# SKIRT/SKIRT9

Measured on AMD Instinct MI355X. Metric: photon packets/s (whole node), 10^6-cell octree, higher is better.
Workload: dtype f64

## Files before the change

skirt9_amd/csrc/pmc_context.h:

```cpp
#ifndef PMC_CONTEXT_H
#define PMC_CONTEXT_H

#include "pmc_device.h"
#include "../../include/pmc_layout.h"
#include "../../include/pmc_tuning.h"
#include <hip/hip_runtime.h>
#include <algorithm>
#include <chrono>
#include <cmath>
#include <cstdio>
#include <rccl/rccl.h>
#include <cstdlib>
#include <cstring>
#include <deque>
#include <atomic>
#include <mutex>
#include <string>
#include <thread>
#include <map>
#include <vector>

extern "C" const char* pmcTune(const char* name);
extern "C" hipError_t pmcUploadScene(int slot, const DevScene* scene, hipStream_t stream);
extern "C" hipError_t pmcConfigureKernels(size_t walkLds, size_t transitionLds);
extern "C" int pmcWalkBlocksPerCU(int gridKind, int kind, int wide, int block, size_t ldsBytes);
extern "C" hipError_t pmcLaunchStatMerge(int slot, int blocks, hipStream_t stream);
extern "C" int pmcPeelBlock(void);
extern "C" int pmcPropBlock(void);
extern "C" hipError_t pmcLaunchWalk(int slot, int gridKind, int flavour, int taskBase, int numTaskRecords, int taskCounter, uint64_t seed, int grid,
                                    int block, size_t ldsBytes, const WalkStreamArgs* tasks, hipStream_t stream);
extern "C" hipError_t pmcLaunchPeel(int slot, int form, int slotBase, int numSlots, const int* list, int cursor, int obs, int sgn, int grid, size_t ldsBytes,
                                    const PeelRec* sortedRec, const unsigned long long* sortedCount, unsigned long long* xcdCursor, hipStream_t stream);
extern "C" int pmcVoroPropWavesPerSimd(void);
extern "C" hipError_t pmcLaunchVoroProp(int slot, const int32_t* list, const unsigned long long* count, unsigned long long* xcdCursor, int segments, uint64_t seed,
                                        int flavour, int grid, hipStream_t stream);
extern "C" int pmcVoroPeelWavesPerSimd(void);
extern "C" hipError_t pmcLaunchVoroPeel(int slot, int rec, int tab, const int32_t* list, const unsigned long long* count, unsigned long long* xcdCursor, int segments,
                                        int severalMedia, int grid, hipStream_t stream);
extern "C" hipError_t pmcLaunchProp(int slot, int wide, int flavour, int checkpoints, int slotBase, int numSlots, const int* list, int cursor, uint64_t seed,
                                    int grid, size_t ldsBytes, const RfLogArgs* rfLog, hipStream_t stream);
extern "C" hipError_t pmcLaunchRfFlush(int slot, const uint32_t* keys, const double* vals, uint32_t* sortedKeys, double* sortedVals, unsigned long long n,
                                       int numParts, void* temp, int numCU, hipStream_t stream);
extern "C" int pmcPeelHasQueues(int form, size_t ldsBytes);
extern "C" int pmcPropHasCheckpoints(int flavour, size_t ldsBytes);
extern "C" int pmcExperimentBuild(void);
extern "C" const unsigned long long* pmcPeelSortedCount(void* temp);
extern "C" size_t pmcPeelSortTempBytes();
extern "C" hipError_t pmcLaunchPeelSortCounts(int slot, int slotBase, int numSlots, PeelSortArgs* ps, PeelRec* const* sorted, int32_t* const* lists, void* const* temp,
                                              int* groups, hipStream_t stream);
extern "C" size_t pmcRfTempBytes(int numParts);
extern "C" int pmcRfMaxParts();
extern "C" hipError_t pmcLaunchDipoleCosines(const double* u, int64_t n, double* out, hipStream_t stream);
extern "C" hipError_t pmcLaunchSourceVelocities(int slot, int source, const double* r, int64_t n, double* out, hipStream_t stream);
extern "C" hipError_t pmcLaunchTransition(int slot, int flavour, int slotBase, int numSlots, int group, uint64_t seed, const int* list, int listLen, int maxBlocks,
                                          size_t ldsBytes, const StatLogArgs* statLog, uint64_t count, hipStream_t stream);
extern "C" hipError_t pmcLaunchLaunch(int slot, int kin, int slotBase, int numSlots, int group, uint64_t first, uint64_t count, uint64_t seed, int initial,
                                      int maxBlocks, size_t ldsBytes, const StatLogArgs* statLog, hipStream_t stream);
extern "C" hipError_t pmcLaunchStatFlush(int slot, const uint32_t* keys, const double* vals, uint32_t* sortedKeys, double* sortedVals, unsigned long long n,
                                         int numParts, void* temp, int numCU, const uint32_t* chunkFill, hipStream_t stream);
extern "C" int pmcStatBucketBits();
extern "C" hipError_t pmcLaunchCycleStart(int slot, int gridKind, int kin, int slotBase, int numSlots, int listCounter, int* listOut, const int* listIn,
                                          int listLen, int maxBlocks, size_t ldsBytes, const PeelSortArgs* sort, hipStream_t stream);
extern "C" hipError_t pmcLaunchTrace(int slot, int gridKind, int wide, int uniform, const double r[3], const double k[3],
                                     const double* kdev, int32_t* m, double* ds, int32_t cap, int32_t* n, size_t ldsBytes,
                                     hipStream_t stream);

void pmcSetError(const std::string& message);
namespace
{
    inline int fail(int code, const std::string& message)
    {
        pmcSetError(message);
        return code;
    }
    inline int hipFail(hipError_t e, const char* what)
    {
        return fail(PMC_ERR_DEVICE, std::string(what) + ": " + hipGetErrorString(e));
    }
}

#define HIP_TRY(call)                                           \
    do                                                          \
// ... 134 lines not shown
```

skirt9_amd/csrc/pmc_device.h:

```cpp
#ifndef PMC_DEVICE_H
#define PMC_DEVICE_H

#include "../../include/pmc.h"
#include <stdint.h>

#define PMC_MAX_INSTRUMENTS 16
#define PMC_MAX_CONTEXTS 6
#define PMC_MAX_LEVEL 20
#define PMC_STAT_CAP 48
#define PMC_STAT_EMISSION_BIN 0x20000000
#define PMC_STAT_POOL_EXHAUSTED 0x40000000

#define PMC_LINK_NONE 0x7FFFFFFFu
#define PMC_LINK_NODE 0x80000000u
#define PMC_LINK_OCTET 0x40000000u
#define PMC_LINK_EXP_BITS 5
#define PMC_LINK_EXP_MASK 31u
#define PMC_LINK_INDEX_MASK 0x1FFFFFFu
#define PMC_LINK_MAX_INDEX ((1u << 25) - 2u)

struct CellRec
{
    double   density;
    uint32_t link[6];
// ... 317 lines not shown
    const unsigned long long* count;
    unsigned long long* xcdCursor;
};
#ifndef PMC_PEEL_TILES
#define PMC_PEEL_TILES 32
#endif
#define PMC_VORO_RUN_UNIT_BITS 27
#define PMC_VORO_RUN_UNIT_MASK 0x07FFFFFFu
#define PMC_VORO_RUN_COUNT_UNKNOWN 31u
#define PMC_VORO_FIRST_SCAN (-1000)
#define PMC_VORO_RUN_PAD 16
#ifndef PMC_VORO_RUN_LANES
#define PMC_VORO_RUN_LANES 2
#endif
#ifndef PMC_VORO_CONES
#define PMC_VORO_CONES 192
#endif
#define PMC_RF_LOG_CHUNK 4096
#define PMC_RF_BUCKET_BITS 13

#define PMC_NUM_COUNTERS 512
#define PMC_CTR_HISTORY 8
#define PMC_CTR_WALKWORK 16
#define PMC_CTR_LIVE(g) (35 + 4 * (g))
#define PMC_CTR_TASK(g, k) (256 + 32 * (g) + (k))
#define PMC_CTR_TASKS_PER_GROUP 32
#define PMC_CTR_LIST(g) PMC_CTR_TASK(g, 30)
#define PMC_CTR_RFLOG(g) PMC_CTR_TASK(g, 31)
#define PMC_CTR_STATLOG(g) (56 + (g))
#define PMC_CTR_HBASE(g) (120 + (g))
#define PMC_CTR_HLIMIT(g) (124 + (g))
#define PMC_MAX_GROUPS 4
#define PMC_CTR_STATFREE(g) (48 + (g))
#define PMC_TRANSITION_ALIGN 1024

#endif
```

skirt9_amd/csrc/pmc_kernels.hip:

```cpp

#include "pmc_device.h"
#include "../../include/pmc_philox.h"
#include <hip/hip_runtime.h>
#include <cstdlib>
#include <cstring>
#include <float.h>
#include <math.h>
#include <algorithm>
#include <mutex>
#include <array>
#include <type_traits>
#include <utility>

#ifndef PMC_WALK_REFILL
    #define PMC_WALK_REFILL 40
#endif
#ifndef PMC_PEEL_REFILL
    #define PMC_PEEL_REFILL 32
#endif
#ifndef PMC_PROP_REFILL
    #define PMC_PROP_REFILL 40
#endif
#ifndef PMC_PEEL_BLOCK
    #define PMC_PEEL_BLOCK 768
// ... 329 lines not shown
{
    WalkStreamArgs ws;
    std::memset(&ws, 0, sizeof(ws));
    if (tasks) ws = *tasks;
    const WalkKernel kernel = gridKind == PMC_GRID_BINTREE ? binWalkKernels[flavour & 7].kernel : walkKernels[(flavour & 7) | (gridKind == PMC_GRID_VORONOI ? 8 : 0)].kernel;
    hipLaunchKernelGGL(kernel, dim3(grid), dim3(block), ldsBytes, stream, slot, taskBase, numTaskRecords, taskCounter, seed, ws);
    return hipGetLastError();
}

extern "C" int pmcVoroPeelWavesPerSimd(void) { return PMC_VPEEL_MIN_WAVES; }
extern "C" hipError_t pmcLaunchVoroPeel(int slot, int rec, int tab, const int32_t* list, const unsigned long long* count, unsigned long long* xcdCursor, int segments,
                                        int severalMedia, int grid, hipStream_t stream)
{
    hipLaunchKernelGGL(severalMedia ? voroPeelKernel<true> : voroPeelKernel<false>, dim3(grid), dim3(256), 0, stream, slot, rec, tab, list, count, xcdCursor,
                       segments);
    return hipGetLastError();
}

extern "C" int pmcVoroPropWavesPerSimd(void) { return PMC_VPROP_MIN_WAVES; }
extern "C" hipError_t pmcLaunchVoroProp(int slot, const int32_t* list, const unsigned long long* count, unsigned long long* xcdCursor, int segments, uint64_t seed,
                                        int flavour, int grid, hipStream_t stream)
{
    hipLaunchKernelGGL(voroPropKernels[flavour & 7], dim3(grid), dim3(256), 0, stream, slot, list, count, xcdCursor, segments, seed);
    return hipGetLastError();
}

constexpr int PEEL_SORT_GROUPS = 1024;
constexpr int PEEL_SORT_PARTS = PMC_PEEL_TILES * PMC_PEEL_TILES;
extern "C" size_t pmcPeelSortTempBytes()
{
    return (size_t(2) * PEEL_SORT_PARTS + 2) * sizeof(unsigned long long) + size_t(PEEL_SORT_GROUPS) * PEEL_SORT_PARTS * sizeof(uint32_t);
}
extern "C" const unsigned long long* pmcPeelSortedCount(void* temp) { return static_cast<const unsigned long long*>(temp) + 2 * PEEL_SORT_PARTS; }
extern "C" hipError_t pmcLaunchPeelSortCounts(int slot, int slotBase, int numSlots, PeelSortArgs* ps, PeelRec* const* sorted, int32_t* const* lists, void* const* temp,
                                              int* groups, hipStream_t stream)
{
    ps->numParts = PEEL_SORT_PARTS;
    const int numLists = ps->numObs + (ps->propIndex >= 0 ? 1 : 0);
    for (int k = 0; k < numLists; ++k)
    {
        unsigned long long* totals = static_cast<unsigned long long*>(temp[k]);
        ps->out[k] = sorted ? sorted[k] : nullptr;
        ps->listOut[k] = lists ? lists[k] : nullptr;
        ps->matrix[k] = reinterpret_cast<uint32_t*>(totals + 2 * PEEL_SORT_PARTS + 2);
        ps->start[k] = totals + PEEL_SORT_PARTS;
    }
    const int tiles = (numSlots + PEEL_SORT_TILE - 1) / PEEL_SORT_TILE;
    *groups = std::max(1, std::min(tiles, PEEL_SORT_GROUPS));
    hipLaunchKernelGGL(peelSortCountKernel, dim3(*groups), dim3(256), 0, stream, slot, slotBase, numSlots, *ps);
    for (int k = 0; k < numLists; ++k)
    {
        unsigned long long* totals = static_cast<unsigned long long*>(temp[k]);
        hipLaunchKernelGGL(peelSortOffsetsKernel, dim3((PEEL_SORT_PARTS + 15) / 16), dim3(256), 0, stream, ps->matrix[k], (uint32_t)*groups, (uint32_t)PEEL_SORT_PARTS, totals);
        hipLaunchKernelGGL(rfScanKernel, dim3(1), dim3(PMC_SCAN_THREADS), 0, stream, totals, totals + PEEL_SORT_PARTS, (uint32_t)PEEL_SORT_PARTS);
    }
    return hipGetLastError();
}

extern "C" hipError_t pmcLaunchPeel(int slot, int form, int slotBase, int numSlots, const int* list, int cursor, int obs, int sgn, int grid, size_t ldsBytes,
                                    const PeelRec* sortedRec, const unsigned long long* sortedCount, unsigned long long* xcdCursor, hipStream_t stream)
{
    if (!(form & 4))
        hipLaunchKernelGGL(peelKernels[form & 3].kernel, dim3(grid), dim3(PMC_PEEL_BLOCK), ldsBytes, stream, slot, slotBase, numSlots, cursor, obs, list);
    else
    {
        const size_t queueOffset = (ldsBytes + 15) & ~size_t(15);
        const PeelSortedArgs sorted = {sortedRec, sortedCount, xcdCursor};
        hipLaunchKernelGGL(peel2Kernels[(form & 1) * 8 + (sgn & 7)].kernel, dim3(grid), dim3(PMC_PEEL_BLOCK), queueOffset + pmcPeelQueueBytes(), stream, slot,
                           slotBase, numSlots, cursor, obs, (int)queueOffset, list, sorted);
    }
    return hipGetLastError();
}

extern "C" hipError_t pmcLaunchProp(int slot, int wide, int flavour, int checkpoints, int slotBase, int numSlots, const int* list, int cursor, uint64_t seed,
                                    int grid, size_t ldsBytes, const RfLogArgs* rfLog, hipStream_t stream)
{
    const PropKernel kernel = propKernels[(flavour & 7) | (wide ? 8 : 0)].kernel;
    const size_t trimOffset = (ldsBytes + 15) & ~size_t(15);
    RfLogArgs none = {nullptr, nullptr, 0ull, 0, 0u};
    hipLaunchKernelGGL(kernel, dim3(grid), dim3(PMC_PROP_BLOCK), checkpoints ? trimOffset + PROP_CKPT_BYTES : ldsBytes, stream, slot, slotBase, numSlots, cursor,
                       seed, checkpoints ? (int)trimOffset : -1, rfLog ? *rfLog : none, list);
    return hipGetLastError();
// ... 146 lines not shown
```

skirt9_amd/csrc/pmc_run.hip:

```cpp
#include "pmc_context.h"

namespace
{
    int allocateSlotArrays(pmc_ctx* ctx, int64_t n);
    void releaseSlots(pmc_ctx* ctx)
    {
        for (void* p : ctx->slotAllocations) hipFree(p);
        ctx->slotAllocations.clear();
        ctx->allocatedSlots = 0;
    }

    int allocateSlots(pmc_ctx* ctx, int64_t n)
    {
        hipSetDevice(ctx->device);
        releaseSlots(ctx);
        ctx->planning = true;
        ctx->plannedBytes = 0;
        int rc = allocateSlotArrays(ctx, n);
        ctx->planning = false;
        if (rc) return rc;
        size_t freeBytes = 0, totalBytes = 0;
        if (!ctx->slotsConfigured && n > (int64_t(1) << 20) && hipMemGetInfo(&freeBytes, &totalBytes) == hipSuccess && ctx->plannedBytes > freeBytes / 2)
        {
            const int64_t less = std::max<int64_t>(int64_t(1) << 20, n / 2);
// ... 100 lines not shown
        for (int32_t** d : tints)
            if ((rc = ctx->allocate<int32_t>(nt, d, false, &own))) return rc;
        if ((rc = ctx->allocate<uint32_t>(size_t(n) / 64 + 64, &K.endedCount, true, &own))) return rc;
        if ((rc = ctx->allocate<int32_t>(2 * size_t(n), &K.liveList, false, &own))) return rc;
        if ((rc = ctx->allocate<uint32_t>(nt, &K.bits, false, &own))) return rc;
    if (ctx->dev.grid_kind == PMC_GRID_OCTREE && (rc = ctx->allocate<uint64_t>(nt, &K.pidx, false, &own))) return rc;
        if (ctx->planning) return PMC_OK;
        A.num_slots = n;
        ctx->allocatedSlots = n;
        ctx->sceneDirty = true;
        return PMC_OK;
    }
}

int pmcAllocateSlots(pmc_ctx* ctx, int64_t n)
{
    return allocateSlots(ctx, n);
}

namespace
{
    struct SegmentPlan
    {
        uint64_t first, count, seed;
        int G;
        int base[PMC_MAX_GROUPS], size[PMC_MAX_GROUPS];
        bool octree;
        int walkFlavour;
        int peelForm;
        bool propCheckpoints;
        int numSortObs, sortObs[PMC_SORT_OBS];
        int propSortIndex, numSortLists;
        PeelSortArgs sortArgs;
        bool sparseLists;
        int listTasksPerLane;
        bool rfLogged, statLogged;
        int rfBuckets, statParts;
        uint32_t rfPadKey;
        unsigned long long rfLogPerSlot, statLogEntries;
        bool poolGrows;
        int statInstruments;
        int launchBlocks, cycleBlocks, transitionBlocks;
        int voroPropGrid, voroPeelGrid, voroPropSegments;
        bool serialWalks, genDump, xcdAffinity, voroPeelKernels, voroPropKernel, voroWalksInSeries;
    };
    struct SegmentRun
    {
        bool active[PMC_MAX_GROUPS], haveWalk[PMC_MAX_GROUPS];
        bool listBuilt[PMC_MAX_GROUPS];
        int listHalf[PMC_MAX_GROUPS];
        bool peelSorted[PMC_MAX_GROUPS];
        bool poolCannotGrow;
        float walkMs, transMs, peelMs, propMs;
        int generations;
    };

    int provisionSlots(pmc_ctx* ctx, uint64_t count, int* numSlots)
    {
        const int64_t want = std::min<int64_t>(ctx->numSlots, (int64_t)std::min<uint64_t>(count, uint64_t(1) << 30));
        bool grow = want > ctx->allocatedSlots;
        if (grow && ctx->allocatedSlots > 0 && ctx->steppedDownFree)
        {
            size_t freeBytes = 0, totalBytes = 0;
            grow = hipMemGetInfo(&freeBytes, &totalBytes) == hipSuccess && freeBytes > ctx->steppedDownFree + ctx->steppedDownFree / 4;
        }
        if (grow)
        {
            HIP_TRY(hipStreamSynchronize(ctx->stream));
            ctx->steppedDownFree = 0;
            int rc = allocateSlots(ctx, want);
            if (rc) return rc;
        }
        *numSlots = (int)std::min<int64_t>(want, ctx->allocatedSlots);
        if (ctx->sceneDirty)
        {
            HIP_TRY(hipStreamSynchronize(ctx->stream));
            HIP_TRY(pmcUploadScene(ctx->slot, &ctx->dev, ctx->stream));
            ctx->sceneDirty = false;
        }
        return PMC_OK;
    }

    SegmentPlan planSegment(const pmc_ctx* ctx, int numSlots, uint64_t first, uint64_t count, uint64_t seed)
    {
// ... 17 lines not shown
        for (int g = 0; g < G; ++g)
        {
            P.base[g] = std::min(numSlots, g * per);
            P.size[g] = std::min(per, numSlots - P.base[g]);
        }
        P.walkFlavour = (D.rf_store ? 1 : 0) | (D.explicit_absorption ? 2 : 0) | (D.num_media > 1 ? 4 : 0);
        P.peelForm = (ctx->wide ? 1 : 0) | (D.num_media > 1 ? 2 : 0);
        if (pmcPeelHasQueues(P.peelForm, ctx->walkLds)) P.peelForm |= 4;
        P.propCheckpoints = pmcPropHasCheckpoints(P.walkFlavour, ctx->walkLds);
        P.propSortIndex = -1;
        if (peelSort && (!P.octree || (P.peelForm & 4)))
        {
            int observers = 0;
            for (int i = 0; i < D.num_instruments; ++i)
                if (!D.inst[i].same_observer)
                {
                    if (observers < PMC_SORT_OBS) P.sortObs[observers] = i;
                    ++observers;
                }
            if (observers <= PMC_SORT_OBS) P.numSortObs = observers;
        }
        if (!P.octree && P.numSortObs > 0 && P.numSortObs < PMC_SORT_OBS && pmcTune("PMC_NO_PROP_SORT") == nullptr) P.propSortIndex = P.numSortObs;
        P.numSortLists = P.numSortObs + (P.propSortIndex >= 0 ? 1 : 0);
        PeelSortArgs& sa = P.sortArgs;
        sa.numObs = P.numSortObs;
        sa.propIndex = P.propSortIndex;
        for (int i = 0; i < 16; ++i) sa.sortIndex[i] = -1;
        for (int k = 0; k < P.numSortObs; ++k) sa.obs[k] = P.sortObs[k], sa.sortIndex[P.sortObs[k]] = (int8_t)k;
        const double gdx = D.gx1 - D.gx0, gdy = D.gy1 - D.gy0, gdz = D.gz1 - D.gz0;
        sa.centre[0] = 0.5 * (D.gx0 + D.gx1), sa.centre[1] = 0.5 * (D.gy0 + D.gy1), sa.centre[2] = 0.5 * (D.gz0 + D.gz1);
        sa.scale = PMC_PEEL_TILES / std::sqrt(gdx * gdx + gdy * gdy + gdz * gdz);
        P.xcdAffinity = pmcTune("PMC_NO_XCD_AFFINITY") == nullptr;
        P.sparseLists = P.octree && pmcTune("PMC_NO_LIVE_LISTS") == nullptr;
        P.listTasksPerLane = 1;
        if (const char* env = pmcTune("PMC_LIST_TASKS_PER_LANE")) P.listTasksPerLane = std::max(1, atoi(env));
        P.voroPeelKernels = D.grid_kind == PMC_GRID_VORONOI && pmcTune("PMC_VORO_NO_PEEL_KERNEL") == nullptr;
        P.voroPropKernel = D.grid_kind == PMC_GRID_VORONOI && D.vgen_run && pmcTune("PMC_VORO_NO_PROP_KERNEL") == nullptr
                           && !(pmcTune("PMC_VORO_PLAIN_PROP_ONLY") && (D.num_media > 1 || D.rf_store || D.explicit_absorption));
        P.voroWalksInSeries = pmcTune("PMC_VORO_WALKS_IN_SERIES") != nullptr;
        P.voroPropSegments = (P.xcdAffinity && pmcTune("PMC_VPROP_XCD_SEGMENTS")) ? 8 : 1;
        int propBlocks = pmcVoroPropWavesPerSimd(), peelBlocks = pmcVoroPeelWavesPerSimd();
        if (const char* v = pmcTune("PMC_VPROP_BLOCKS_PER_CU")) propBlocks = std::max(1, atoi(v));
        if (const char* v = pmcTune("PMC_VPEEL_BLOCKS_PER_CU")) peelBlocks = std::max(1, atoi(v));
        P.voroPropGrid = ctx->numCU * propBlocks, P.voroPeelGrid = ctx->numCU * peelBlocks;
        const int64_t rfKeys = P.octree ? int64_t(D.cell_slots) * D.rf_num_lambda : ctx->rfSize;
        const int64_t rfParts = (rfKeys + (int64_t(1) << PMC_RF_BUCKET_BITS) - 1) >> PMC_RF_BUCKET_BITS;
        P.rfLogged = D.rf_store && P.octree && rfParts <= pmcRfMaxParts() && pmcTune("PMC_RF_ATOMICS") == nullptr;
        if (D.rf_store && P.octree && rfParts > pmcRfMaxParts())
        {
            static std::atomic<bool> said{false};
            if (!said.exchange(true))
                fprintf(stderr, "libpmc: the radiation field table has %lld entries, more than the log's counting sort partitions (%d x %d): contributions are added atomically\n",
                        (long long)rfKeys, pmcRfMaxParts(), 1 << PMC_RF_BUCKET_BITS);
        }
        P.rfBuckets = P.rfLogged ? int(rfParts) : 0;
        P.rfPadKey = uint32_t(P.rfBuckets) << PMC_RF_BUCKET_BITS;
        P.rfLogPerSlot = 128ull;
        if (const char* env = pmcTune("PMC_RF_LOG_PER_SLOT")) P.rfLogPerSlot = std::max(1, atoi(env));
        const int statBits = pmcStatBucketBits();
        P.statParts = int((D.stat_acc_records + (int64_t(1) << statBits) - 1) >> statBits);
        P.statLogged = D.any_stats && D.stat_acc_records > 0 && P.statParts <= pmcRfMaxParts() && pmcTune("PMC_STAT_ATOMICS") == nullptr;
        unsigned long long entries = (128ull << 20);
        if (const char* env = pmcTune("PMC_STAT_LOG_ENTRIES")) entries = std::max(1, atoi(env));
        P.statLogEntries = std::max<unsigned long long>((entries + PMC_RF_LOG_CHUNK - 1) / PMC_RF_LOG_CHUNK, 1ull) * PMC_RF_LOG_CHUNK;
        for (int i = 0; i < D.num_instruments; ++i) P.statInstruments += D.inst[i].record_stats ? 1 : 0;
        P.poolGrows = D.any_stats && ctx->statPoolBlocks > 0 && pmcTune("PMC_STAT_POOL_NO_GROWTH") == nullptr;
// ... 219 lines not shown
            D.stat_pool_first[h] = first;
            D.stat_pool_count[h] = count;
            first += count;
        }
        freeNow[g] += (unsigned long long)add;
        HIP_TRY(hipMemcpy(ctr + PMC_CTR_STATFREE(0), freeNow, sizeof(freeNow), hipMemcpyHostToDevice));
        ctx->release(D.stat_pool_bin, own), ctx->release(D.stat_pool_w, own), ctx->release(D.stat_pool_next, own), ctx->release(D.stat_pool_free, own);
        ctx->release(ctx->statPoolIota, own);
        D.stat_pool_bin = bin, D.stat_pool_w = w, D.stat_pool_next = next, D.stat_pool_free = stack;
        ctx->statPoolIota = iota;
        ctx->statPoolBlocks = old + add;
        ctx->readback[g].statFreeBlocks = freeNow[g];
        ctx->statPoolGrowths += 1;
        HIP_TRY(pmcUploadScene(ctx->slot, &D, ctx->stream));
        HIP_TRY(hipStreamSynchronize(ctx->stream));
        return PMC_OK;
    }

    int enqueueOctreeWalks(pmc_ctx* ctx, const SegmentPlan& P, const SegmentRun& S, int g, const int* listIn, int listLen)
    {
        const DevScene& D = ctx->dev;
        hipStream_t sg = ctx->groupStream[g], sp = P.serialWalks ? sg : ctx->peelStream[g];
        const int numTasks = listIn ? listLen : P.size[g];
        const int peelLanes = pmcPeelBlock() * P.listTasksPerLane, propLanes = pmcPropBlock() * P.listTasksPerLane;
        const int peelGrid = listIn ? std::max(1, std::min(ctx->peelGrid, (numTasks + peelLanes - 1) / peelLanes)) : ctx->peelGrid;
        const int propGrid = listIn ? std::max(1, std::min(ctx->grid, (numTasks + propLanes - 1) / propLanes)) : ctx->grid;
        HIP_TRY(hipStreamWaitEvent(sp, ctx->evA[g], 0));
        for (int i = 0; i < D.num_instruments; ++i)
            if (!D.inst[i].same_observer)
            {
                int k = -1;
                for (int q = 0; q < P.numSortObs; ++q)
                    if (P.sortObs[q] == i) k = q;
                const bool sorted = S.peelSorted[g] && !listIn && k >= 0;
                HIP_TRY(pmcLaunchPeel(ctx->slot, P.peelForm, P.base[g], numTasks, sorted ? nullptr : listIn, PMC_CTR_TASK(g, 1 + i), i, (int)D.inst[i].sgn, peelGrid,
                                      ctx->walkLds, sorted ? ctx->peelRec[g][k] : nullptr, sorted ? pmcPeelSortedCount(ctx->peelTemp[g][k]) : nullptr,
                                      sorted && P.xcdAffinity ? cursorSet(ctx, g, k) : nullptr, sp));
            }
        HIP_TRY(hipEventRecord(ctx->evJoin[g], sp));
        RfLogArgs log = {ctx->rfKeys[g][0], ctx->rfVals[g][0], P.rfLogged ? ctx->rfCap[g] : 0ull, PMC_CTR_RFLOG(g), P.rfPadKey};
        if (P.serialWalks) HIP_TRY(hipEventRecord(ctx->evProp[g], sg));
        HIP_TRY(pmcLaunchProp(ctx->slot, ctx->wide, P.walkFlavour, P.propCheckpoints, P.base[g], numTasks, listIn, PMC_CTR_TASK(g, 0), P.seed, propGrid, ctx->walkLds,
                              &log, sg));
        if (!P.serialWalks) HIP_TRY(hipEventRecord(ctx->evProp[g], sg));
        HIP_TRY(hipStreamWaitEvent(sg, ctx->evJoin[g], 0));
        return PMC_OK;
    }

    int enqueueGenericWalks(pmc_ctx* ctx, const SegmentPlan& P, const SegmentRun& S, int g)
    {
        const DevScene& D = ctx->dev;
        hipStream_t sg = ctx->groupStream[g];
        auto ownPeel = [&](int k) { return P.voroPeelKernels && D.vobs_of_inst[P.sortObs[k]] >= 0; };
        WalkStreamArgs tasks;
        std::memset(&tasks, 0, sizeof(tasks));
        bool streamEmpty = false;
        if (S.peelSorted[g])
        {
            tasks.numLists = P.numSortObs;
            for (int k = 0; k < P.numSortObs; ++k)
                tasks.rec[k] = 1 + P.sortObs[k], tasks.list[k] = ctx->peelList[g][k], tasks.count[k] = pmcPeelSortedCount(ctx->peelTemp[g][k]);
            tasks.xcdCursor = P.xcdAffinity ? cursorSet(ctx, g, 0) : nullptr;
            if (P.propSortIndex >= 0)
                tasks.propList = ctx->peelList[g][P.propSortIndex], tasks.propCount = pmcPeelSortedCount(ctx->peelTemp[g][P.propSortIndex]);
            bool left = false;
            for (int k = 0; k < P.numSortObs; ++k)
                if (ownPeel(k))
// ... 7 lines not shown
                tasks.propCount = zeroCount(ctx);
            }
            else
                left = true;
            streamEmpty = !left;
        }
        if (!streamEmpty)
            HIP_TRY(pmcLaunchWalk(ctx->slot, D.grid_kind, P.walkFlavour, P.base[g], P.size[g], PMC_CTR_TASK(g, 0), P.seed, ctx->grid, ctx->block, ctx->walkLds,
                                  S.peelSorted[g] ? &tasks : nullptr, sg));
        if (!S.peelSorted[g]) return PMC_OK;
        bool anyPeel = false;
        for (int k = 0; k < P.numSortObs; ++k) anyPeel = anyPeel || ownPeel(k);
        const bool side = anyPeel && P.voroPropKernel && P.propSortIndex >= 0 && !P.serialWalks && !P.voroWalksInSeries;
        hipStream_t sp = side ? ctx->peelStream[g] : sg;
        if (side) HIP_TRY(hipStreamWaitEvent(sp, ctx->evA[g], 0));
        for (int k = 0; k < P.numSortObs; ++k)
            if (ownPeel(k))
                HIP_TRY(pmcLaunchVoroPeel(ctx->slot, 1 + P.sortObs[k], D.vobs_of_inst[P.sortObs[k]], ctx->peelList[g][k], pmcPeelSortedCount(ctx->peelTemp[g][k]),
                                          cursorSet(ctx, g, 1 + k), P.xcdAffinity ? 8 : 1, D.num_media > 1 ? 1 : 0, P.voroPeelGrid, sp));
        if (side)
        {
            HIP_TRY(hipEventRecord(ctx->evJoin[g], sp));
            HIP_TRY(hipStreamWaitEvent(sg, ctx->evJoin[g], 0));
        }
        return PMC_OK;
    }

    int enqueueCycleStart(pmc_ctx* ctx, const SegmentPlan& P, SegmentRun& S, int g, bool initial, const int* listIn, int listLen)
    {
        DevScene& D = ctx->dev;
        hipStream_t sg = ctx->groupStream[g];
        unsigned long long* ctr = D.counters;
        GroupReadback& rb = ctx->readback[g];
        const bool buildList = P.sparseLists && !initial && (listIn || rb.live < (unsigned long long)(P.size[g] / 2));
        if (listIn) S.listHalf[g] ^= 1;
        int* const listOut = D.tasks.liveList + int64_t(S.listHalf[g]) * D.slots.num_slots + P.base[g];
        const bool sortNow = P.numSortObs > 0 && !buildList && !listIn;
        PeelSortArgs sortArgs = P.sortArgs;
        sortArgs.cap = (uint32_t)ctx->peelCap[g];
        int sortGroups = 0;
        if (sortNow)
            HIP_TRY(pmcLaunchPeelSortCounts(ctx->slot, P.base[g], P.size[g], &sortArgs, P.octree ? ctx->peelRec[g] : nullptr, P.octree ? nullptr : ctx->peelList[g],
                                            ctx->peelTemp[g], &sortGroups, sg));
        HIP_TRY(pmcLaunchCycleStart(ctx->slot, D.grid_kind, D.kin, P.base[g], P.size[g], buildList ? PMC_CTR_LIST(g) : -1, listOut, listIn, listLen,
                                    sortNow ? sortGroups : P.cycleBlocks, ctx->walkLds, sortNow ? &sortArgs : nullptr, sg));
        S.peelSorted[g] = sortNow;
        S.listBuilt[g] = buildList;
        HIP_TRY(hipEventRecord(ctx->evC[g], sg));
        const size_t word = sizeof(unsigned long long);
        HIP_TRY(hipMemcpyAsync(&rb.live, ctr + PMC_CTR_LIVE(g), word, hipMemcpyDeviceToHost, sg));
        if (P.rfLogged && !initial) HIP_TRY(hipMemcpyAsync(&rb.rfLogFill, ctr + PMC_CTR_RFLOG(g), word, hipMemcpyDeviceToHost, sg));
        if (ctx->progress) HIP_TRY(hipMemcpyAsync(&rb.historyCursor, ctr + PMC_CTR_HISTORY, word, hipMemcpyDeviceToHost, sg));
        if (P.statLogged && !initial && ctx->statCap[g]) HIP_TRY(hipMemcpyAsync(&rb.statLogFill, ctr + PMC_CTR_STATLOG(g), word, hipMemcpyDeviceToHost, sg));
        if (P.poolGrows) HIP_TRY(hipMemcpyAsync(&rb.statFreeBlocks, ctr + PMC_CTR_STATFREE(g), word, hipMemcpyDeviceToHost, sg));
        return PMC_OK;
    }

    int enqueueGeneration(pmc_ctx* ctx, const SegmentPlan& P, SegmentRun& S, int g, bool initial)
    {
        const DevScene& D = ctx->dev;
        hipStream_t sg = ctx->groupStream[g];
        unsigned long long* ctr = D.counters;
        GroupReadback& rb = ctx->readback[g];
        int* const listIn = (!initial && S.listBuilt[g]) ? D.tasks.liveList + int64_t(S.listHalf[g]) * D.slots.num_slots + P.base[g] : nullptr;
        const int listLen = listIn ? int(rb.live) : 0;
        if (initial)
        {
            if (g > 0) HIP_TRY(hipStreamWaitEvent(sg, ctx->evStart, 0));
            HIP_TRY(hipEventRecord(ctx->evB[g], sg));
            HIP_TRY(pmcLaunchLaunch(ctx->slot, ctx->dev.kin, P.base[g], P.size[g], g, P.first, P.count, P.seed, 1, (P.size[g] + 255) / 256, ctx->launchLds, nullptr, sg));
            return enqueueCycleStart(ctx, P, S, g, initial, listIn, listLen);
        }
        if (P.poolGrows)
        {
            const int64_t need = int64_t(rb.live) * P.statInstruments, freeBlocks = int64_t(rb.statFreeBlocks);
            const bool inUse = freeBlocks < int64_t(D.stat_pool_count[g]) || D.min_scatt_events > 16;
            if (inUse && freeBlocks < need && !S.poolCannotGrow)
            {
                const int64_t before = ctx->statPoolBlocks;
                if (int rc = growStatPool(ctx, g, need)) return rc;
                S.poolCannotGrow = ctx->statPoolBlocks == before;
            }
        }
        if (int rc = rfFlush(ctx, P, g, rb.rfLogFill)) return rc;
        rb.rfLogFill = 0;
        if (rb.statLogFill > ctx->statCap[g] / 2)
        {
            if (int rc = statFlush(ctx, P, g, rb.statLogFill, sg)) return rc;
            rb.statLogFill = 0;
        }
        HIP_TRY(hipMemsetAsync(ctr + PMC_CTR_TASK(g, 0), 0, PMC_CTR_TASKS_PER_GROUP * sizeof(unsigned long long), sg));
        if (ctx->xcdCursors) HIP_TRY(hipMemsetAsync(cursorSet(ctx, g, 0), 0, (PMC_SORT_OBS + 1) * 8 * sizeof(unsigned long long), sg));
        HIP_TRY(hipEventRecord(ctx->evA[g], sg));
        if (int rc = P.octree ? enqueueOctreeWalks(ctx, P, S, g, listIn, listLen) : enqueueGenericWalks(ctx, P, S, g)) return rc;
        S.haveWalk[g] = true;
        HIP_TRY(hipEventRecord(ctx->evB[g], sg));
        HIP_TRY(hipMemsetAsync(ctr + PMC_CTR_LIVE(g), 0, sizeof(unsigned long long), sg));
        const StatLogArgs statLog = statLogOf(ctx, P, g);
        HIP_TRY(pmcLaunchTransition(ctx->slot, (ctx->dev.any_dipole ? 1 : 0) | (ctx->dev.kin ? 2 : 0), P.base[g], P.size[g], g, P.seed, listIn, listLen, P.transitionBlocks, ctx->transitionLds, &statLog, P.count, sg));
        if (!listIn)
            HIP_TRY(pmcLaunchLaunch(ctx->slot, ctx->dev.kin, P.base[g], P.size[g], g, P.first, P.count, P.seed, 0, P.launchBlocks, ctx->launchLds, &statLog, sg));
        return enqueueCycleStart(ctx, P, S, g, initial, listIn, listLen);
    }

    int drive(pmc_ctx* ctx, const SegmentPlan& P, SegmentRun& S)
    {
        auto lastReport = std::chrono::steady_clock::now();
        const auto segmentStart = lastReport;
        uint64_t reported = 0;
        int remaining = 0;
        for (int g = 0; g < P.G; ++g)
        {
            S.active[g] = P.size[g] > 0;
            remaining += S.active[g] ? 1 : 0;
        }
        for (int g = 0; g < P.G; ++g)
            if (S.active[g])
                if (int rc = enqueueGeneration(ctx, P, S, g, true)) return rc;
        for (int g = 0; remaining > 0; g = (g + 1) % P.G)
        {
            if (!S.active[g]) continue;
            HIP_TRY(hipStreamSynchronize(ctx->groupStream[g]));
            GroupReadback& rb = ctx->readback[g];
            float ms = 0, walkOfGen = 0;
            if (S.haveWalk[g])
            {
// ... 3 lines not shown
                if (P.octree)
                {
                    HIP_TRY(hipEventElapsedTime(&ms, ctx->evA[g], ctx->evJoin[g]));
                    S.peelMs += ms;
                    if (P.serialWalks)
                        HIP_TRY(hipEventElapsedTime(&ms, ctx->evProp[g], ctx->evB[g]));
                    else
                        HIP_TRY(hipEventElapsedTime(&ms, ctx->evA[g], ctx->evProp[g]));
                    S.propMs += ms;
                }
            }
            HIP_TRY(hipEventElapsedTime(&ms, ctx->evB[g], ctx->evC[g]));
            S.transMs += ms;
            if (rb.live == 0)
            {
                if (int rc = rfFlush(ctx, P, g, rb.rfLogFill)) return rc;
                rb.rfLogFill = 0;
                S.active[g] = false;
                --remaining;
                continue;
            }
            ++S.generations;
            if (ctx->progress)
            {
                const auto now = std::chrono::steady_clock::now();
                if (std::chrono::duration<double>(now - lastReport).count() >= ctx->progressInterval)
                {
                    lastReport = now;
                    reported = std::max<uint64_t>(reported, std::min<uint64_t>(rb.historyCursor, P.count));
                    ctx->progress(ctx->progressUser, reported, P.count);
                }
            }
            if (P.genDump)
                fprintf(stderr, "PMC_GEN %d group %d live %llu walk_ms %.3f transition_ms %.3f at_ms %.3f\n", S.generations, g, rb.live,
                        S.haveWalk[g] ? walkOfGen : 0.f, ms, 1e3 * std::chrono::duration<double>(std::chrono::steady_clock::now() - segmentStart).count());
            if (int rc = enqueueGeneration(ctx, P, S, g, false)) return rc;
        }
        return PMC_OK;
    }

    int finish(pmc_ctx* ctx, const SegmentPlan& P)
    {
        if (P.statLogged)
            for (int g = 0; g < P.G; ++g)
                if (int rc = statFlush(ctx, P, g, ctx->readback[g].statLogFill, ctx->groupStream[g])) return rc;
        if (P.rfLogged || P.statLogged)
            for (int g = 0; g < P.G; ++g) HIP_TRY(hipStreamSynchronize(ctx->groupStream[g]));
        if (ctx->dev.stat_acc_records) HIP_TRY(pmcLaunchStatMerge(ctx->slot, ctx->numCU * 8, ctx->stream));
        HIP_TRY(hipEventRecord(ctx->evStop, ctx->stream));
        HIP_TRY(hipEventSynchronize(ctx->evStop));
        HIP_TRY(hipEventElapsedTime(&ctx->totalMs, ctx->evStart, ctx->evStop));
        return PMC_OK;
    }

    int abandon(pmc_ctx* ctx, int code)
    {
        hipDeviceSynchronize();
        if (ctx->dev.stat_acc_records) hipMemset(ctx->dev.stat_acc, 0, size_t(ctx->dev.stat_acc_records) * 8 * sizeof(double));
        ctx->timed = false;
        return code;
    }

    int checkKernelErrors(pmc_ctx* ctx)
    {
        const unsigned long long* ctr = ctx->dev.counters;
        {
            unsigned long long tail[3] = {0, 0, 0};
            HIP_TRY(hipMemcpy(tail, ctr + 5, sizeof(tail), hipMemcpyDeviceToHost));
// ... 54 lines not shown
```

skirt9_amd/csrc/pmc_transition.inc:

```

    struct DustLds
    {
        const double* lamb;
        const double* sext;
        const double* ssca;
        const double* asym;
        const double* src;
        double* sed;
        unsigned long long* hotKey;
        double* hotVal;
    };
    constexpr int HOT_BINS = 256;

    struct PhaseHG
    {
        double g;
        double onePlusG2;
        double twoG;
        double norm;
        __device__ __forceinline__ explicit PhaseHG(double asym) : g(asym), onePlusG2(1. + asym * asym), twoG(2. * asym), norm((1. - asym) * (1. + asym)) {}
        __device__ __forceinline__ double kernel(double c) const { return onePlusG2 - twoG * c; }
        __device__ __forceinline__ double value(double c) const
        {
            const double t = kernel(c);
// ... 1667 lines not shown
        PMC_T_PROF_END(200);
        addCounters(S, cnt, lane);
    }
    __global__ __launch_bounds__(256, PMC_LAUNCH_MIN_WAVES) void launchKernel(const int sceneSlot, const int slotBase, const int numSlots, const int group,
                                                        const uint64_t first, const uint64_t count, const uint64_t seed, const int initial,
                                                        const StatLogArgs statLog)
    {
        launchBody<false>(sceneSlot, slotBase, numSlots, group, first, count, seed, initial, statLog);
    }
    __global__ __launch_bounds__(256, PMC_LAUNCH_MIN_WAVES) void launchKinKernel(const int sceneSlot, const int slotBase, const int numSlots, const int group,
                                                        const uint64_t first, const uint64_t count, const uint64_t seed, const int initial,
                                                        const StatLogArgs statLog)
    {
        launchBody<true>(sceneSlot, slotBase, numSlots, group, first, count, seed, initial, statLog);
    }

    template<int GRID, bool KIN = false>
    __global__ __launch_bounds__(256, PMC_CYCLE_MIN_WAVES) void cycleStartKernel(const int sceneSlot, const int slotBase, const int numSlots,
                                                                                 const int listCounter, int* const listOut,
                                                                                 const int* const listIn, const int listLen, const PeelSortArgs ps)
    {
        const DevScene& S = c_scene[sceneSlot];
        extern __shared__ double lds[];
        const int tid = threadIdx.x;
        const int lane = tid & 63;
        if (GRID == GRID_TREE) requireLdsBaseZero(lds);
        stageGrid<GRID>(S, lds, tid, blockDim.x);
        __syncthreads();
        const GridLds G = makeGridLds(S, lds);
        const SlotArrays& A = S.slots;
        Counters cnt = {0, 0, 0, 0, 0};
        const int slotEnd = slotBase + numSlots;
        const bool sparse = GRID == GRID_TREE && listIn != nullptr;
        if (ps.numObs > 0 && !sparse)
        {
            uint32_t* const cur = reinterpret_cast<uint32_t*>(reinterpret_cast<char*>(lds) + ps.ldsOffset);
            const int numLists = ps.numObs + (ps.propIndex >= 0 ? 1 : 0);
            for (int k = 0; k < numLists; ++k)
                for (uint32_t p = tid; p < ps.numParts; p += blockDim.x)
                    cur[(uint32_t)k * ps.numParts + p] = (uint32_t)ps.start[k][p] + ps.matrix[k][(size_t)blockIdx.x * ps.numParts + p];
            __syncthreads();
            const int tiles = (numSlots + PEEL_SORT_TILE - 1) / PEEL_SORT_TILE;
            for (int t = blockIdx.x; t < tiles; t += gridDim.x)
                for (int i = t * PEEL_SORT_TILE + tid; i < (t + 1) * PEEL_SORT_TILE && i < numSlots; i += blockDim.x)
                {
                    const int slot = slotBase + i;
                    const int md = A.mode[slot];
                    if (md & MODE_ALIVE) startCycleWalks<GRID, KIN>(S, G, cnt, slot, md, &ps, cur);
                }
        }
        else
        {
            const int end = sparse ? listLen : numSlots;
            for (int i0 = blockIdx.x * blockDim.x; i0 < end; i0 += gridDim.x * blockDim.x)
            {
                const int i = i0 + tid;
                const int slot = sparse ? (i < listLen ? listIn[i] : -1) : slotBase + i;
                const int md = (slot >= 0 && slot < slotEnd) ? A.mode[slot] : 0;
                if (md & MODE_ALIVE) startCycleWalks<GRID, KIN>(S, G, cnt, slot, md);
                if (GRID == GRID_TREE && listCounter >= 0)
                {
                    const unsigned long long m = __ballot((md & MODE_ALIVE) != 0);
                    if (m)
                    {
                        unsigned long long at = 0;
                        if (lane == __ffsll((long long)m) - 1) at = atomicAdd(S.counters + listCounter, (unsigned long long)__popcll(m));
                        at = __shfl(at, __ffsll((long long)m) - 1, 64);
                        if (md & MODE_ALIVE) listOut[(int)at + __popcll(m & ((1ull << lane) - 1ull))] = slot;
                    }
                }
            }
        }
        const unsigned long long v = waveSum(cnt.paths);
        if (lane == 0 && v) atomicAdd(S.counters + 1, v);
    }

    __global__ __launch_bounds__(256) void peelSortCountKernel(const int sceneSlot, const int slotBase, const int numSlots, const PeelSortArgs ps)
    {
        const DevScene& S = c_scene[sceneSlot];
        const SlotArrays& A = S.slots;
        __shared__ uint32_t h[PMC_SORT_OBS * PMC_PEEL_TILES * PMC_PEEL_TILES];
        const int tid = threadIdx.x;
        const int numLists = ps.numObs + (ps.propIndex >= 0 ? 1 : 0);
        for (uint32_t p = tid; p < (uint32_t)numLists * ps.numParts; p += blockDim.x) h[p] = 0u;
        __syncthreads();
        const int tiles = (numSlots + PEEL_SORT_TILE - 1) / PEEL_SORT_TILE;
        for (int t = blockIdx.x; t < tiles; t += gridDim.x)
            for (int i = t * PEEL_SORT_TILE + tid; i < (t + 1) * PEEL_SORT_TILE && i < numSlots; i += blockDim.x)
            {
                const int slot = slotBase + i;
                const int md = A.mode[slot];
                if (!(md & MODE_ALIVE)) continue;
                const double x = A.rx[slot], y = A.ry[slot], z = A.rz[slot];
                for (int k = 0; k < ps.numObs; ++k)
                    if (((uint32_t)md >> (8 + ps.obs[k])) & 1u) atomicAdd(&h[(uint32_t)k * ps.numParts + peelTile(ps, S.inst[ps.obs[k]], x, y, z)], 1u);
                if (ps.propIndex >= 0)
                    atomicAdd(&h[(uint32_t)ps.propIndex * ps.numParts + propSortKey(S, x, y, z, A.kx[slot], A.ky[slot], A.kz[slot])], 1u);
            }
        __syncthreads();
        for (int k = 0; k < numLists; ++k)
            for (uint32_t p = tid; p < ps.numParts; p += blockDim.x) ps.matrix[k][(size_t)blockIdx.x * ps.numParts + p] = h[(uint32_t)k * ps.numParts + p];
    }
    __global__ __launch_bounds__(256) void peelSortOffsetsKernel(uint32_t* __restrict__ matrix, const uint32_t groups, const uint32_t numParts,
                                                                 unsigned long long* __restrict__ totals)
    {
        __shared__ uint32_t part[16][17];
        const uint32_t pl = threadIdx.x & 15u, run = threadIdx.x >> 4;
        const uint32_t p = blockIdx.x * 16u + pl;
        const uint32_t rows = (groups + 15u) / 16u;
        const uint32_t b0 = run * rows, b1 = b0 + rows < groups ? b0 + rows : groups;
        uint32_t sum = 0u;
        if (p < numParts)
            for (uint32_t b = b0; b < b1; ++b) sum += matrix[(size_t)b * numParts + p];
        part[run][pl] = sum;
        __syncthreads();
        uint32_t before = 0u, all = 0u;
        for (uint32_t r = 0; r < 16u; ++r)
        {
            const uint32_t v = part[r][pl];
            if (r < run) before += v;
            all += v;
        }
        if (p < numParts)
// ... 11 lines not shown
```

Baseline: 209.5 million.

## Allow peel sorting together with sparse live lists and add hysteresis to list use

```diff
diff --git a/skirt9_amd/csrc/pmc_context.h b/skirt9_amd/csrc/pmc_context.h
--- a/skirt9_amd/csrc/pmc_context.h
+++ b/skirt9_amd/csrc/pmc_context.h
@@ -46,8 +46,8 @@
 extern "C" int pmcExperimentBuild(void);
 extern "C" const unsigned long long* pmcPeelSortedCount(void* temp);
 extern "C" size_t pmcPeelSortTempBytes();
-extern "C" hipError_t pmcLaunchPeelSortCounts(int slot, int slotBase, int numSlots, PeelSortArgs* ps, PeelRec* const* sorted, int32_t* const* lists, void* const* temp,
-                                              int* groups, hipStream_t stream);
+extern "C" hipError_t pmcLaunchPeelSortCounts(int slot, int slotBase, int numSlots, const int* listIn, int listLen, PeelSortArgs* ps, PeelRec* const* sorted,
+                                              int32_t* const* lists, void* const* temp, int* groups, hipStream_t stream);
 extern "C" size_t pmcRfTempBytes(int numParts);
 extern "C" int pmcRfMaxParts();
 extern "C" hipError_t pmcLaunchDipoleCosines(const double* u, int64_t n, double* out, hipStream_t stream);
diff --git a/skirt9_amd/csrc/pmc_device.h b/skirt9_amd/csrc/pmc_device.h
--- a/skirt9_amd/csrc/pmc_device.h
+++ b/skirt9_amd/csrc/pmc_device.h
@@ -373,6 +373,9 @@
 #define PMC_CTR_HLIMIT(g) (124 + (g))
 #define PMC_MAX_GROUPS 4
 #define PMC_CTR_STATFREE(g) (48 + (g))
+#ifndef PMC_LIST_BELOW_EIGHTHS
+#define PMC_LIST_BELOW_EIGHTHS 6
+#endif
 #define PMC_TRANSITION_ALIGN 1024
 
 #endif
diff --git a/skirt9_amd/csrc/pmc_kernels.hip b/skirt9_amd/csrc/pmc_kernels.hip
--- a/skirt9_amd/csrc/pmc_kernels.hip
+++ b/skirt9_amd/csrc/pmc_kernels.hip
@@ -385,8 +385,8 @@
     return (size_t(2) * PEEL_SORT_PARTS + 2) * sizeof(unsigned long long) + size_t(PEEL_SORT_GROUPS) * PEEL_SORT_PARTS * sizeof(uint32_t);
 }
 extern "C" const unsigned long long* pmcPeelSortedCount(void* temp) { return static_cast<const unsigned long long*>(temp) + 2 * PEEL_SORT_PARTS; }
-extern "C" hipError_t pmcLaunchPeelSortCounts(int slot, int slotBase, int numSlots, PeelSortArgs* ps, PeelRec* const* sorted, int32_t* const* lists, void* const* temp,
-                                              int* groups, hipStream_t stream)
+extern "C" hipError_t pmcLaunchPeelSortCounts(int slot, int slotBase, int numSlots, const int* listIn, int listLen, PeelSortArgs* ps, PeelRec* const* sorted,
+                                              int32_t* const* lists, void* const* temp, int* groups, hipStream_t stream)
 {
     ps->numParts = PEEL_SORT_PARTS;
     const int numLists = ps->numObs + (ps->propIndex >= 0 ? 1 : 0);
@@ -398,9 +398,9 @@
         ps->matrix[k] = reinterpret_cast<uint32_t*>(totals + 2 * PEEL_SORT_PARTS + 2);
         ps->start[k] = totals + PEEL_SORT_PARTS;
     }
-    const int tiles = (numSlots + PEEL_SORT_TILE - 1) / PEEL_SORT_TILE;
+    const int tiles = ((listIn ? listLen : numSlots) + PEEL_SORT_TILE - 1) / PEEL_SORT_TILE;
     *groups = std::max(1, std::min(tiles, PEEL_SORT_GROUPS));
-    hipLaunchKernelGGL(peelSortCountKernel, dim3(*groups), dim3(256), 0, stream, slot, slotBase, numSlots, *ps);
+    hipLaunchKernelGGL(peelSortCountKernel, dim3(*groups), dim3(256), 0, stream, slot, slotBase, numSlots, listIn, listLen, *ps);
     for (int k = 0; k < numLists; ++k)
     {
         unsigned long long* totals = static_cast<unsigned long long*>(temp[k]);
diff --git a/skirt9_amd/csrc/pmc_run.hip b/skirt9_amd/csrc/pmc_run.hip
--- a/skirt9_amd/csrc/pmc_run.hip
+++ b/skirt9_amd/csrc/pmc_run.hip
@@ -156,7 +156,8 @@
         int numSortObs, sortObs[PMC_SORT_OBS];
         int propSortIndex, numSortLists;
         PeelSortArgs sortArgs;
-        bool sparseLists;
+        bool sparseLists, sparseSort;
+        int listBelowEighths;
         int listTasksPerLane;
         bool rfLogged, statLogged;
         int rfBuckets, statParts;
@@ -172,8 +173,10 @@
     {
         bool active[PMC_MAX_GROUPS], haveWalk[PMC_MAX_GROUPS];
         bool listBuilt[PMC_MAX_GROUPS];
+        bool listUsed[PMC_MAX_GROUPS];
         int listHalf[PMC_MAX_GROUPS];
         bool peelSorted[PMC_MAX_GROUPS];
+        bool peelSortedWalks[PMC_MAX_GROUPS];
         bool poolCannotGrow;
         float walkMs, transMs, peelMs, propMs;
         int generations;
@@ -257,6 +260,9 @@
         sa.scale = PMC_PEEL_TILES / std::sqrt(gdx * gdx + gdy * gdy + gdz * gdz);
         P.xcdAffinity = pmcTune("PMC_NO_XCD_AFFINITY") == nullptr;
         P.sparseLists = P.octree && pmcTune("PMC_NO_LIVE_LISTS") == nullptr;
+        P.sparseSort = pmcTune("PMC_NO_SPARSE_SORT") == nullptr;
+        P.listBelowEighths = PMC_LIST_BELOW_EIGHTHS;
+        if (const char* v = pmcTune("PMC_LIST_BELOW_EIGHTHS")) P.listBelowEighths = std::min(8, std::max(0, atoi(v)));
         P.listTasksPerLane = 1;
         if (const char* env = pmcTune("PMC_LIST_TASKS_PER_LANE")) P.listTasksPerLane = std::max(1, atoi(env));
         P.voroPeelKernels = D.grid_kind == PMC_GRID_VORONOI && pmcTune("PMC_VORO_NO_PEEL_KERNEL") == nullptr;
@@ -542,7 +548,7 @@
                 int k = -1;
                 for (int q = 0; q < P.numSortObs; ++q)
                     if (P.sortObs[q] == i) k = q;
-                const bool sorted = S.peelSorted[g] && !listIn && k >= 0;
+                const bool sorted = S.peelSorted[g] && k >= 0;
                 HIP_TRY(pmcLaunchPeel(ctx->slot, P.peelForm, P.base[g], numTasks, sorted ? nullptr : listIn, PMC_CTR_TASK(g, 1 + i), i, (int)D.inst[i].sgn, peelGrid,
                                       ctx->walkLds, sorted ? ctx->peelRec[g][k] : nullptr, sorted ? pmcPeelSortedCount(ctx->peelTemp[g][k]) : nullptr,
                                       sorted && P.xcdAffinity ? cursorSet(ctx, g, k) : nullptr, sp));
@@ -616,15 +622,15 @@
         hipStream_t sg = ctx->groupStream[g];
         unsigned long long* ctr = D.counters;
         GroupReadback& rb = ctx->readback[g];
-        const bool buildList = P.sparseLists && !initial && (listIn || rb.live < (unsigned long long)(P.size[g] / 2));
+        const bool buildList = P.sparseLists && !initial && (listIn || rb.live < (unsigned long long)P.size[g]);
         if (listIn) S.listHalf[g] ^= 1;
         int* const listOut = D.tasks.liveList + int64_t(S.listHalf[g]) * D.slots.num_slots + P.base[g];
-        const bool sortNow = P.numSortObs > 0 && !buildList && !listIn;
+        const bool sortNow = P.numSortObs > 0 && (P.sparseSort || (!buildList && !listIn));
         PeelSortArgs sortArgs = P.sortArgs;
         sortArgs.cap = (uint32_t)ctx->peelCap[g];
         int sortGroups = 0;
         if (sortNow)
-            HIP_TRY(pmcLaunchPeelSortCounts(ctx->slot, P.base[g], P.size[g], &sortArgs, P.octree ? ctx->peelRec[g] : nullptr, P.octree ? nullptr : ctx->peelList[g],
+            HIP_TRY(pmcLaunchPeelSortCounts(ctx->slot, P.base[g], P.size[g], listIn, listLen, &sortArgs, P.octree ? ctx->peelRec[g] : nullptr, P.octree ? nullptr : ctx->peelList[g],
                                             ctx->peelTemp[g], &sortGroups, sg));
         HIP_TRY(pmcLaunchCycleStart(ctx->slot, D.grid_kind, D.kin, P.base[g], P.size[g], buildList ? PMC_CTR_LIST(g) : -1, listOut, listIn, listLen,
                                     sortNow ? sortGroups : P.cycleBlocks, ctx->walkLds, sortNow ? &sortArgs : nullptr, sg));
@@ -646,7 +652,9 @@
         hipStream_t sg = ctx->groupStream[g];
         unsigned long long* ctr = D.counters;
         GroupReadback& rb = ctx->readback[g];
-        int* const listIn = (!initial && S.listBuilt[g]) ? D.tasks.liveList + int64_t(S.listHalf[g]) * D.slots.num_slots + P.base[g] : nullptr;
+        const bool useList = !initial && S.listBuilt[g] && (S.listUsed[g] || rb.live * 8ull < (unsigned long long)P.size[g] * (unsigned long long)P.listBelowEighths);
+        S.listUsed[g] = useList;
+        int* const listIn = useList ? D.tasks.liveList + int64_t(S.listHalf[g]) * D.slots.num_slots + P.base[g] : nullptr;
         const int listLen = listIn ? int(rb.live) : 0;
         if (initial)
         {
@@ -676,6 +684,7 @@
         HIP_TRY(hipMemsetAsync(ctr + PMC_CTR_TASK(g, 0), 0, PMC_CTR_TASKS_PER_GROUP * sizeof(unsigned long long), sg));
         if (ctx->xcdCursors) HIP_TRY(hipMemsetAsync(cursorSet(ctx, g, 0), 0, (PMC_SORT_OBS + 1) * 8 * sizeof(unsigned long long), sg));
         HIP_TRY(hipEventRecord(ctx->evA[g], sg));
+        S.peelSortedWalks[g] = S.peelSorted[g];
         if (int rc = P.octree ? enqueueOctreeWalks(ctx, P, S, g, listIn, listLen) : enqueueGenericWalks(ctx, P, S, g)) return rc;
         S.haveWalk[g] = true;
         HIP_TRY(hipEventRecord(ctx->evB[g], sg));
@@ -745,8 +754,9 @@
                 }
             }
             if (P.genDump)
-                fprintf(stderr, "PMC_GEN %d group %d live %llu walk_ms %.3f transition_ms %.3f at_ms %.3f\n", S.generations, g, rb.live,
-                        S.haveWalk[g] ? walkOfGen : 0.f, ms, 1e3 * std::chrono::duration<double>(std::chrono::steady_clock::now() - segmentStart).count());
+                fprintf(stderr, "PMC_GEN %d group %d live %llu walk_ms %.3f transition_ms %.3f at_ms %.3f list %d sorted %d\n", S.generations, g, rb.live,
+                        S.haveWalk[g] ? walkOfGen : 0.f, ms, 1e3 * std::chrono::duration<double>(std::chrono::steady_clock::now() - segmentStart).count(),
+                        S.listUsed[g] ? 1 : 0, S.peelSortedWalks[g] ? 1 : 0);
             if (int rc = enqueueGeneration(ctx, P, S, g, false)) return rc;
         }
         return PMC_OK;
diff --git a/skirt9_amd/csrc/pmc_transition.inc b/skirt9_amd/csrc/pmc_transition.inc
--- a/skirt9_amd/csrc/pmc_transition.inc
+++ b/skirt9_amd/csrc/pmc_transition.inc
@@ -1723,7 +1723,16 @@
         Counters cnt = {0, 0, 0, 0, 0};
         const int slotEnd = slotBase + numSlots;
         const bool sparse = GRID == GRID_TREE && listIn != nullptr;
-        if (ps.numObs > 0 && !sparse)
+        const int end = sparse ? listLen : numSlots;
+        auto appendLive = [&](const int slot, const bool alive) {
+            const unsigned long long m = __ballot(alive);
+            if (!m) return;
+            unsigned long long at = 0;
+            if (lane == __ffsll((long long)m) - 1) at = atomicAdd(S.counters + listCounter, (unsigned long long)__popcll(m));
+            at = __shfl(at, __ffsll((long long)m) - 1, 64);
+            if (alive) listOut[(int)at + __popcll(m & ((1ull << lane) - 1ull))] = slot;
+        };
+        if (ps.numObs > 0)
         {
             uint32_t* const cur = reinterpret_cast<uint32_t*>(reinterpret_cast<char*>(lds) + ps.ldsOffset);
             const int numLists = ps.numObs + (ps.propIndex >= 0 ? 1 : 0);
@@ -1731,42 +1740,60 @@
                 for (uint32_t p = tid; p < ps.numParts; p += blockDim.x)
                     cur[(uint32_t)k * ps.numParts + p] = (uint32_t)ps.start[k][p] + ps.matrix[k][(size_t)blockIdx.x * ps.numParts + p];
             __syncthreads();
-            const int tiles = (numSlots + PEEL_SORT_TILE - 1) / PEEL_SORT_TILE;
+            const int tiles = (end + PEEL_SORT_TILE - 1) / PEEL_SORT_TILE;
+            const bool listing = GRID == GRID_TREE && listCounter >= 0;
             for (int t = blockIdx.x; t < tiles; t += gridDim.x)
-                for (int i = t * PEEL_SORT_TILE + tid; i < (t + 1) * PEEL_SORT_TILE && i < numSlots; i += blockDim.x)
-                {
-                    const int slot = slotBase + i;
-                    const int md = A.mode[slot];
-                    if (md & MODE_ALIVE) startCycleWalks<GRID, KIN>(S, G, cnt, slot, md, &ps, cur);
-                }
+            {
+                const int tileEnd = min((t + 1) * PEEL_SORT_TILE, end);
+                int at = 0;
+                if (listing)
+                {
+                    int n = 0;
+                    for (int i0 = t * PEEL_SORT_TILE; i0 < tileEnd; i0 += blockDim.x)
+                    {
+                        const int i = i0 + tid;
+                        const int slot = i < end ? (sparse ? listIn[i] : slotBase + i) : -1;
+                        const int md = (slot >= 0 && slot < slotEnd) ? A.mode[slot] : 0;
+                        n += __popcll(__ballot((md & MODE_ALIVE) != 0));
+                    }
+                    unsigned long long first = 0;
+                    if (lane == 0 && n) first = atomicAdd(S.counters + listCounter, (unsigned long long)n);
+                    at = (int)__shfl(first, 0, 64);
+                }
+                for (int i0 = t * PEEL_SORT_TILE; i0 < tileEnd; i0 += blockDim.x)
+                {
+                    const int i = i0 + tid;
+                    const int slot = i < end ? (sparse ? listIn[i] : slotBase + i) : -1;
+                    const int md = (slot >= 0 && slot < slotEnd) ? A.mode[slot] : 0;
+                    const bool alive = (md & MODE_ALIVE) != 0;
+                    if (listing)
+                    {
+                        const unsigned long long m = __ballot(alive);
+                        const int to = at + __popcll(m & ((1ull << lane) - 1ull));
+                        if (alive && to < numSlots) listOut[to] = slot;
+                        at += __popcll(m);
+                    }
+                    if (alive) startCycleWalks<GRID, KIN>(S, G, cnt, slot, md, &ps, cur);
+                }
+            }
         }
         else
         {
-            const int end = sparse ? listLen : numSlots;
             for (int i0 = blockIdx.x * blockDim.x; i0 < end; i0 += gridDim.x * blockDim.x)
             {
                 const int i = i0 + tid;
                 const int slot = sparse ? (i < listLen ? listIn[i] : -1) : slotBase + i;
                 const int md = (slot >= 0 && slot < slotEnd) ? A.mode[slot] : 0;
                 if (md & MODE_ALIVE) startCycleWalks<GRID, KIN>(S, G, cnt, slot, md);
-                if (GRID == GRID_TREE && listCounter >= 0)
-                {
-                    const unsigned long long m = __ballot((md & MODE_ALIVE) != 0);
-                    if (m)
-                    {
-                        unsigned long long at = 0;
-                        if (lane == __ffsll((long long)m) - 1) at = atomicAdd(S.counters + listCounter, (unsigned long long)__popcll(m));
-                        at = __shfl(at, __ffsll((long long)m) - 1, 64);
-                        if (md & MODE_ALIVE) listOut[(int)at + __popcll(m & ((1ull << lane) - 1ull))] = slot;
-                    }
-                }
+                if (GRID == GRID_TREE && listCounter >= 0) appendLive(slot, (md & MODE_ALIVE) != 0);
             }
         }
         const unsigned long long v = waveSum(cnt.paths);
         if (lane == 0 && v) atomicAdd(S.counters + 1, v);
     }
 
-    __global__ __launch_bounds__(256) void peelSortCountKernel(const int sceneSlot, const int slotBase, const int numSlots, const PeelSortArgs ps)
+    __global__ __launch_bounds__(256) void peelSortCountKernel(const int sceneSlot, const int slotBase, const int numSlots, const int* const listIn, const int listLen,
+                                                               const PeelSortArgs ps)
     {
         const DevScene& S = c_scene[sceneSlot];
         const SlotArrays& A = S.slots;
@@ -1775,11 +1802,13 @@
         const int numLists = ps.numObs + (ps.propIndex >= 0 ? 1 : 0);
         for (uint32_t p = tid; p < (uint32_t)numLists * ps.numParts; p += blockDim.x) h[p] = 0u;
         __syncthreads();
-        const int tiles = (numSlots + PEEL_SORT_TILE - 1) / PEEL_SORT_TILE;
+        const int end = listIn ? listLen : numSlots;
+        const int tiles = (end + PEEL_SORT_TILE - 1) / PEEL_SORT_TILE;
         for (int t = blockIdx.x; t < tiles; t += gridDim.x)
-            for (int i = t * PEEL_SORT_TILE + tid; i < (t + 1) * PEEL_SORT_TILE && i < numSlots; i += blockDim.x)
-            {
-                const int slot = slotBase + i;
+            for (int i = t * PEEL_SORT_TILE + tid; i < (t + 1) * PEEL_SORT_TILE && i < end; i += blockDim.x)
+            {
+                const int slot = listIn ? listIn[i] : slotBase + i;
+                if (slot < slotBase || slot >= slotBase + numSlots) continue;
                 const int md = A.mode[slot];
                 if (!(md & MODE_ALIVE)) continue;
                 const double x = A.rx[slot], y = A.ry[slot], z = A.rz[slot];
```

Result: no change. 210.1 million, median of 5 (+0.3%).
